# MinghanLi/MDQE_CVPR2023

Measured on AMD Instinct MI355X. Metric: frames/sec (eval-only) R50 OVIS 360p 4-frame clip, higher is better.
Workload: dtype f32; 1 GPU; R50_ovis_360 eval-only, H2D included: 120 synthetic 360x640 u8 frames/GPU/step from pinned host memory, 4-frame clips stride 1, 30-frame windows, one model(inputs) call per video; random-init weights, calibrated class logits (DESIGN.md §5); frames_per_gpu=120, instances_out=10, tracked_instances=7, gemm=exact fp32 MFMA, hw_queues=4, ranks_seen=1, parallelism=single GPU

## Files before the change

include/mdqe_hip.h:

```cpp
#ifndef MDQE_HIP_H
#define MDQE_HIP_H
#include <stdint.h>

#ifdef __cplusplus
extern "C" {
#endif

#define MDQE_OK 0
#define MDQE_EINVAL 1
#define MDQE_ELAUNCH 2
#define MDQE_ENULL 3
#define MDQE_ESTATE 4

#define MDQE_ACT_NONE 0
#define MDQE_ACT_RELU 1
#define MDQE_ACT_GELU 2
#define MDQE_ACT_SIGMOID 3
#define MDQE_ACT_TANH 4

#define MDQE_ABI_VERSION 6
int mdqe_abi_version(void);
int mdqe_version(void);
const char* mdqe_strerror(int code);

// ... 116 lines not shown
int mdqe_stem_conv_f32(const void* frames, int is_u8, long frame_stride, int NI, int h, int w, int Hp, int Wp,
                       const float* mean3_host, const float* std3_host, const float* wk, const float* bias, float* out,
                       void* stream);

int mdqe_maxpool3x3s2_nhwc_f32(const float* x, float* y, int NI, int H, int W, int C, void* stream);

int mdqe_upsample_nearest_add_nhwc_f32(const float* a, const float* b, float* y, int NI, int H, int W, int Hb, int Wb,
                                       int C, void* stream);

int mdqe_dwconv5x5_nhwc_f32(const float* x, const float* wt, const float* bias, float* y, int NI, int H, int W, int C,
                            int up2, const float* tw, const float* tb, void* stream);

int mdqe_dwconv5x5_c256_f32(const float* x, const float* wt, const float* bias, float* y, int NI, int H, int W, void* stream);
int mdqe_dwconv5x5_up2_c256_f32(const float* x, const float* wt, const float* bias, const float* tw, const float* tb, float* y,
                                int NI, int Hs, int Ws, void* stream);

int mdqe_trk_siou_f32(const float* saved, long saved_stride, int n_saved, const float* inp, long inp_stride,
                      int n_in, long n, float* out3, void* stream);
int mdqe_trk_accumulate_f32(float* sum, long sum_stride, float* cnt, long cnt_stride, const float* src,
                            long src_stride, long n, int nf, const int* r_host, const int* c_host, int count,
                            void* stream);
int mdqe_trk_siou_host_f32(const float* saved, long saved_stride, int n_saved, const float* inp, long inp_stride,
                           int n_in, long n, float* acc, unsigned* ticket, unsigned long long* out_host,
                           unsigned seq, void* stream);
int mdqe_trk_wait_counts(const unsigned long long* out_host, int n_out, unsigned seq, int spin_us, float* counts, void* stream);

int mdqe_trk_window_mean_f32(const float* sum, const float* cnt, long hw, int mem_len, int n, int nf, long f0,
                             float* out, void* stream);
int mdqe_trk_carry_f32(float* sum, float* cnt, long hw, int mem_len, int n, int k, long src0, float* carry, void* stream);

// ... 17 lines not shown
                            float* carry, float* out_cls, int* n, int* ln, void* stream);

int mdqe_clip_assoc_f32(const float* emb, int Q, int E, const int* fidx, int Bc, int T, int ct, float wdw, int nb,
                        int* idx_out, void* stream);
int mdqe_clip_gather_init_f32(const float* content, const float* coords, const int* fidx, const int* idx, int Bc, int T,
                              int Q, int C, int ct, float* x, float* ref, float* xinst, void* stream);
int mdqe_box_refine_f32(const float* delta, const float* prev, int Bc, int T, int Q, int t0, int t1, float* boxes,
                        float* ibox, void* stream);
int mdqe_add_rows_f32(const float* a, long lda, const float* b, long ldb, float* out, long ldo, long rows, int C, void* stream);
int mdqe_time_fuse_f32(const float* w, const float* x, int Bc, int T, int Q, int C, float* out, const float* pos,
                       float* out_plus_pos, void* stream);
int mdqe_box_head_refine_f32(const float* h, long ldh, const float* W, const float* bias, const float* prev, int Bc, int T, int Q, int K,
                             int t0, int t1, float* boxes, float* ibox, void* stream);
int mdqe_time_fuse_dot_f32(const float* xw, const float* wt, const float* bt, const float* src, int Bc, int T, int Q, int C, float* out,
                           void* stream);

int mdqe_clip_select_f32(const float* cls, const float* emb, int B, int Q, int K, int C, float thr, int max_keep,
                         int* order_ws, int* n_thr_ws, float* inv_norm_ws, float* sim_ws, int* kept, int* n_keep, void* stream);
long mdqe_dyn_mask_workspace_floats(int n_rows, int T, int H, int W);
int mdqe_dyn_mask_nms_f32(const float* coef, const int* kept, const float* feats, int B, int Q, int M, int T, int H, int W,
                          const int* row0_host, const int* n_host, const int* f0_host, float* logits, float* soft_h,
                          float* hard_h, float* part, float* gram, float* stats, float* mi, void* stream);
long mdqe_nms_workspace_floats(int n_max);
int mdqe_clip_finalize_f32(const float* cls, const float* emb, const int* kept, const float* stats, const float* mi, int B,
                           int Q, int K, int C, float thr, const int* row0_host, const int* n_host, int* sel, int* n_sel,
                           float* out, void* stream);
int mdqe_rows_gather_f32(const float* src, const int* idx_dev, int n, long len, float* out, void* stream);

int mdqe_mask_row_stats_f32(const float* logits, int n, int T, int H, int W, int t_step, float* stats5,
                            float* soft_h, float* hard_h, void* stream);
// ... 76 lines not shown
```

mdqe_cvpr2023_amd/_lib.py:

```python
import ctypes
import os
from ctypes import c_char_p, c_float, c_int, c_void_p

_HERE = os.path.dirname(os.path.abspath(__file__))
LIB_PATH = os.environ.get("MDQE_HIP_LIB") or os.path.join(_HERE, "csrc", "libmdqe_hip.so")

from ctypes import c_long
i, f, p, l = c_int, c_float, c_void_p, c_long

SIGNATURES = {
    "mdqe_msda_forward_f32": [p, p, p, p, p, i, i, i, i, i, i, i, p, p],
    "mdqe_msda_backward_f32": [p, p, p, p, p, p, i, i, i, i, i, i, i, p, p, p, p],
    "mdqe_msda_forward_f64": [p, p, p, p, p, i, i, i, i, i, i, i, p, p],
    "mdqe_msda_backward_f64": [p, p, p, p, p, p, i, i, i, i, i, i, i, p, p, p, p],
    "mdqe_msda_forward_grouped_f32": [p, p, p, p, p, i, i, i, i, i, i, i, i, f, p, p],
    "mdqe_msda_fused_f32": [p, l, l, p, p, l, p, l, p, l, i, i, p, p, p, p, i, i, i, i, i, i, i, f, p, l, l, p],
    "mdqe_trk_siou_f32": [p, l, i, p, l, i, l, p, p],
    "mdqe_trk_accumulate_f32": [p, l, p, l, p, l, l, i, p, p, i, p],
    "mdqe_trk_window_mean_f32": [p, p, l, i, i, i, l, p, p],
    "mdqe_trk_carry_f32": [p, p, l, i, i, i, l, p, p],
    "mdqe_lsap_f64": [p, i, i, i, p, p, p],
    "mdqe_tracker_create": [i, i, i, i, i, i, f, p],
    "mdqe_tracker_destroy": [p],
    "mdqe_tracker_state": [p, p, p, p],
    "mdqe_tracker_overlap": [p, i, i, p, p, p, p],
    "mdqe_tracker_decide": [p, i, i, i, p, p, p, p, p, p, p, p, p, p],
    "mdqe_tracker_result": [p, i, p, p, p, p],
    "mdqe_tracker_update": [p, p, p, l, i, i, i, p, p, p, p, l, p, p, p],
    "mdqe_tracker_update_many": [p, p, p, l, i, p, p, p, p, p, p, p, p, p, p, p, p],
    "mdqe_tracker_get_result": [p, i, p, p, l, p, p, p, p, p, p],
    "mdqe_clip_assoc_f32": [p, i, i, p, i, i, i, f, i, p, p],
    "mdqe_clip_gather_init_f32": [p, p, p, p, i, i, i, i, i, p, p, p, p],
    "mdqe_box_refine_f32": [p, p, i, i, i, i, i, p, p, p],
    "mdqe_add_rows_f32": [p, l, p, l, p, l, l, i, p],
    "mdqe_time_fuse_f32": [p, p, i, i, i, i, p, p, p, p],
    "mdqe_box_head_refine_f32": [p, l, p, p, p, i, i, i, i, i, i, p, p, p],
    "mdqe_time_fuse_dot_f32": [p, p, p, p, i, i, i, i, p, p],
    "mdqe_clip_select_f32": [p, p, i, i, i, i, f, i, p, p, p, p, p, p, p],
    "mdqe_dyn_mask_nms_f32": [p, p, p, i, i, i, i, i, i, p, p, p, p, p, p, p, p, p, p, p],
    "mdqe_clip_finalize_f32": [p, p, p, p, p, i, i, i, i, f, p, p, p, p, p, p],
    "mdqe_rows_gather_f32": [p, p, i, l, p, p],
    "mdqe_mha_small_f32": [p, l, p, l, p, l, i, i, i, i, p],
    "mdqe_query_select_f32": [p, i, i, i, i, i, p, p, p],
    "mdqe_sample_levels_mean_f32": [p, i, l, i, p, i, p, p, p, i, p, p],
    "mdqe_image_mask_stats_f32": [p, i, i, i, i, i, i, p, p],
    "mdqe_image_final_masks_u8": [p, i, p, i, i, i, i, i, i, i, p, p],
    "mdqe_final_masks_rle": [p, i, p, i, i, i, i, i, i, i, i, i, p, p, p],
    "mdqe_final_masks_u8": [p, i, p, i, i, i, i, i, i, i, i, p, l, i, p],
    "mdqe_final_masks_rle_geom": [p, i, p, i, i, i, i, i, i, i, i, i, p, p, p, p],
    "mdqe_final_masks_u8_geom": [p, i, p, i, i, i, i, i, i, i, i, p, l, i, p, p],
    "mdqe_final_label_map_u8": [p, i, p, i, i, i, i, i, i, i, i, p, i, p, p],
    "mdqe_render_overlay_u8": [p, i, l, i, i, p, i, i, i, p, i, i, p, i, p],
# ... 46 lines not shown
    "mdqe_gemm_ln_f32": [p, l, p, p, p, l, i, i, i, p, l, p, p, f, p],
    "mdqe_gemm_ln2_f32": [p, l, p, p, p, l, i, i, i, p, l, p, p, p, p, p, l, f, p],
    "mdqe_gemm_nt_side_f32": [p, l, p, p, p, l, i, i, i, p, p, i, p, p],
    "mdqe_gemm_nt_cat2_f32": [p, l, i, p, l, i, i, i, i, i, i, i, p, p, p, l, i, i, p],
    "mdqe_gemm_nt_pix_f32": [p, l, i, i, i, i, i, i, i, p, p, p, l, i, i, p],
    "mdqe_groupnorm_nhwc_f32": [p, l, l, p, l, l, i, i, i, i, p, p, f, i, p, p],
    "mdqe_resize_pil_bilinear_u8": [p, l, i, i, i, i, i, i, p, p, p, i, p, p, p, i, p, p],
    "mdqe_yuv420sp_to_rgb_u8": [p, l, l, p, l, l, i, i, i, i, i, i, i, p, p],
    "mdqe_stem_im2col_f32": [p, i, l, i, i, i, i, i, p, p, p, p],
    "mdqe_stem_conv_f32": [p, i, l, i, i, i, i, i, p, p, p, p, p, p],
    "mdqe_maxpool3x3s2_nhwc_f32": [p, p, i, i, i, i, p],
    "mdqe_upsample_nearest_add_nhwc_f32": [p, p, p, i, i, i, i, i, i, p],
    "mdqe_dwconv5x5_nhwc_f32": [p, p, p, p, i, i, i, i, i, p, p, p],
    "mdqe_dwconv5x5_c256_f32": [p, p, p, p, i, i, i, p],
    "mdqe_dwconv5x5_up2_c256_f32": [p, p, p, p, p, p, i, i, i, p],
}


ABI_VERSION = 6


class LibraryMissing(RuntimeError):
    pass


class MdqeError(RuntimeError):
    pass


_lib = None
# ... 71 lines not shown
```

mdqe_cvpr2023_amd/csrc/clip_ops.hip:

```cpp
#include "common.h"

#include <math.h>

template <int E>
__global__ void __launch_bounds__(64)
clip_assoc_kernel(const float* __restrict__ emb, const int* __restrict__ fidx, int T, int Q, int ct, float wdw, int nb,
                  int* __restrict__ idx) {
  extern __shared__ __attribute__((aligned(16))) float sE[];
  const int bt = blockIdx.y, b = bt / T, t = bt % T;
  const int k = blockIdx.x * 64 + threadIdx.x;
  const float* et = emb + (long)fidx[b * T + t] * Q * E;
  const float* ec = emb + (long)fidx[b * T + ct] * Q * E;
  for (int i = threadIdx.x; i < Q * (E / 4); i += 64)
    *reinterpret_cast<f32x4*>(sE + i * 4) = *reinterpret_cast<const f32x4*>(et + i * 4);
  __syncthreads();
  if (k >= Q) return;
  float c[E];
#pragma unroll
  for (int e = 0; e < E; e += 4) {
    const f32x4 v = *reinterpret_cast<const f32x4*>(ec + (long)k * E + e);
    c[e] = v[0]; c[e + 1] = v[1]; c[e + 2] = v[2]; c[e + 3] = v[3];
  }
  const float w = wdw * (float)abs(t - ct);
  const int ki = k / nb, kj = k % nb;
// ... 231 lines not shown
    }
  }
  if (lane == 0) *reinterpret_cast<f32x4*>(ibox + i * 4) = f32x4{(x0 + x1) / 2.f, (y0 + y1) / 2.f, x1 - x0, y1 - y0};
}

extern "C" int mdqe_box_head_refine_f32(const float* h, long ldh, const float* W, const float* bias, const float* prev, int Bc, int T,
                                        int Q, int K, int t0, int t1, float* boxes, float* ibox, void* stream) {
  MDQE_REQUIRE(Bc >= 0 && T > 0 && Q > 0 && K > 0 && K % 256 == 0 && ldh >= K && ldh % 4 == 0 && t0 >= 0 && t0 < t1);
  if (Bc == 0) return MDQE_OK;
  MDQE_CHECK_PTR(h); MDQE_CHECK_PTR(W); MDQE_CHECK_PTR(bias); MDQE_CHECK_PTR(prev); MDQE_CHECK_PTR(boxes); MDQE_CHECK_PTR(ibox);
  MDQE_REQUIRE((((uintptr_t)h | (uintptr_t)W | (uintptr_t)prev | (uintptr_t)boxes | (uintptr_t)ibox) & 15) == 0);
  mdqe_clear_error();
  const long n = (long)Bc * Q;
  hipLaunchKernelGGL(box_head_refine_kernel, dim3((unsigned)((n + 3) / 4)), dim3(256), 0, (hipStream_t)stream, h, ldh, W, bias, prev, T, Q, K,
                     t0, t1 < T ? t1 : T, n, boxes, ibox);
  return mdqe_launch_status();
}

__global__ void __launch_bounds__(256)
time_fuse_dot_kernel(const float* __restrict__ xw, const float* __restrict__ wt, const float* __restrict__ bt,
                     const float* __restrict__ src, int T, int Q, long n, float* __restrict__ out) {
  constexpr int C = 256, TMAX = 8;
  const int lane = threadIdx.x & 63;
  const long i = (long)blockIdx.x * 4 + (threadIdx.x >> 6);
  if (i >= n) return;
  const long b = i / Q;
  const int q = (int)(i % Q);
  const f32x4 w = *reinterpret_cast<const f32x4*>(wt + lane * 4);
  float tw[TMAX];
  float m = -INFINITY;
// ... 477 lines not shown
```

mdqe_cvpr2023_amd/engine.py:

```python
import contextlib
import math
import os
from types import SimpleNamespace as NS

import numpy as np
import torch
import torch.nn.functional as F

from . import ops
from .config import MDQEConfig
from .params import ALIASES, RESNET_BLOCKS, msda_dir_grid


def _fold_bn(sd, p, eps=1e-5):
    scale = sd[p + ".norm.weight"] * (sd[p + ".norm.running_var"] + eps).rsqrt()
    shift = sd[p + ".norm.bias"] - sd[p + ".norm.running_mean"] * scale
    return sd[p + ".weight"] * scale.view(-1, 1, 1, 1), shift


GEO_CACHE = max(1, int(os.environ.get("MDQE_GEO_CACHE", "16")))
STEM_FUSED = os.environ.get("MDQE_STEM_FUSED", "1") != "0"
SWIN_FUSED = os.environ.get("MDQE_SWIN_FUSED", "1") != "0"
RESNET_CAT = os.environ.get("MDQE_RESNET_CAT", "1") != "0"

# ... 296 lines not shown


def box_cxcywh_to_xyxy(b):
    cx, cy, w, h = b.unbind(-1)
    return torch.stack([cx - 0.5 * w, cy - 0.5 * h, cx + 0.5 * w, cy + 0.5 * h], -1)


def box_xyxy_to_cxcywh(b):
    x0, y0, x1, y1 = b.unbind(-1)
    return torch.stack([(x0 + x1) / 2, (y0 + y1) / 2, x1 - x0, y1 - y0], -1)


INST_STREAMS = {}
DEC_TWO_STREAMS = os.environ.get("MDQE_DEC_TWO_STREAMS", "1") != "0"
DEC_FUSED = os.environ.get("MDQE_DEC_FUSED", "1") != "0"


class Engine:
    def __init__(self, cfg: MDQEConfig, state_dict, device="cuda", backbone_fn=None, only_backbone=False):
        self.cfg = cfg
        self.P = Packed(state_dict, cfg, device, only_backbone=only_backbone)
        self.dev = self.P.dev
        self.backbone_fn = backbone_fn
        self._geo = {}
        self.precision_map = os.environ.get("MDQE_PRECISION_MAP", "")
        if self.precision_map not in ("", "reference", "autocast_f16"):
            raise ValueError("MDQE_PRECISION_MAP: '' (exact fp32 everywhere), 'reference' or 'autocast_f16', not %r" % self.precision_map)

    def amp(self):
        if self.precision_map == "reference" and self.dev.type == "cuda":
# ... 146 lines not shown
    def _mask_features(self, enc, geo, out=None):
        mh, cfg = self.P.mh, self.cfg
        NI, N, C = enc.shape
        lv = [enc[:, geo.starts[l]:geo.starts[l] + geo.hw[l]].view(NI, geo.shapes[l][0], geo.shapes[l][1], C) for l in range(3)]
        x = ops.conv2d_nhwc(lv[2], *mh.lay1, 1, 1)
        x = ops.groupnorm_nhwc(x, 8, *mh.gn1, act="gelu", out=x).view(x.shape)
        for i, f in ((2, lv[1]), (3, lv[0])):
            cur = ops.conv2d_nhwc(f, *getattr(mh, f"ad{i - 1}"), 1, 0)
            x = ops.upsample_nearest_add(cur, x, out=cur)
            x = ops.conv2d_nhwc(x, *getattr(mh, f"lay{i}"), 1, 1)
            x = ops.groupnorm_nhwc(x, 8, *getattr(mh, f"gn{i}"), act="gelu", out=x).view(x.shape)
        o1, o2 = mh.out_lay1, mh.out_lay2
        y = ops.dwconv5x5(x, o1.dw, o1.db)
        y = ops.linear(y.view(-1, C), o1.pw, o1.pb).view(x.shape)
        y = ops.groupnorm_nhwc(y, 32, o1.g, o1.beta, act="relu", out=y).view(x.shape)
        z = ops.dwconv5x5(y, o2.dw, o2.db, up2=True, tw=mh.tw, tb=mh.tb)
        Md = o2.pw.shape[0]
        if out is not None and (tuple(out.shape) != (NI, z.shape[1], z.shape[2], Md) or not out.is_contiguous()):
            raise RuntimeError("mask_features: out must be a contiguous [NI, Hm, Wm, M] tensor")
        z2 = ops.linear(z.view(-1, C), o2.pw, o2.pb, out=None if out is None else out.view(-1, Md)).view(NI, z.shape[1], z.shape[2], Md)
        return ops.groupnorm_nhwc(z2, 32 if Md % 32 == 0 else 24, o2.g, o2.beta, act="relu", out=z2).view(z2.shape)

    def _mlp(self, x, layers, last_act=None, out=None):
        n = len(layers)
        for i, (w, b) in enumerate(layers):
            x = ops.linear(x, w, b, act="gelu" if i < n - 1 else last_act, out=out if i == n - 1 else None)
        return x

    def frame_queries(self, enc, geo, out=None):
        cfg = self.cfg
        NI, N, C = enc.shape
        H, W = geo.shapes[0]
        nb = cfg.n_bins
        o_coords, o_content, o_emb = out if out is not None else (None, None, None)
        with self.amp():
# ... 34 lines not shown
    def decode_clips(self, cache, starts, T, geo, two_streams=True):
        P, cfg = self.P, self.cfg
        Bc = len(starts)
        fidx_h = np.asarray([[a + t for t in range(T)] for a in starts], dtype=np.int32).reshape(Bc, T)
        lo, hi = int(fidx_h.min()), int(fidx_h.max()) + 1
        if lo > 0 or hi < cache["content"].shape[0]:
            cache = {k: v[lo:hi] for k, v in cache.items() if k in ("coords", "content", "emb", "vals")}
            fidx_h = fidx_h - lo
        fidx = self._to_dev_i32(fidx_h)
        content, vals = cache["content"], cache["vals"]
        Q, C = content.shape[1], content.shape[2]
        nh, N = cfg.nheads, geo.N
        D, Tc = C // nh, cfg.n_frames
        ct = int((T - 1) / 2)
        idx = ops.clip_assoc(cache["emb"], fidx, ct, cfg.window_inter_frame_asso / 2, cfg.n_bins) if T > 1 else None
        x, ref, x_inst = ops.clip_gather_init(content, cache["coords"], fidx, idx, ct)
        BT = Bc * T
        fused = DEC_FUSED
        small = fused and C == 256

        def refine(z, prev, zn=None):
            z = ops.layernorm(z, *P.dec_norm) if zn is None else zn
            if small:
                h = ops.linear(ops.linear(z, *P.bbox_embed[0], act="gelu"), *P.bbox_embed[1], act="gelu")
                return ops.box_head_refine(h, *P.bbox_embed[2], prev, Bc, T, Q, t0, t1)
            return ops.box_refine(self._mlp(z, P.bbox_embed), prev, Bc, T, Q, t0, t1)

        def qkv(sa, z, box, B_):
            if fused:
                o = ops.linear_side(z, sa.wqkv, sa.bqkv_pos, box, sa.side_w, 2 * C)
                return ops.mha_small(o[:, :2 * C], o[:, 2 * C:], B_, Q, C, nh)
            zp = ops.add_rows(z, ops.linear(box, *P.p2p))
            return ops.mha_small(ops.linear(zp, sa.wqk, sa.bqk), ops.linear(z, sa.wv, sa.bv), B_, Q, C, nh)

        def qproj(m, z, box):
            if fused:
                return ops.linear_side(z, m.wq, m.bq_pos, box, m.side_w, m.wq.shape[0])
            return ops.linear(ops.add_rows(z, ops.linear(box, *P.p2p)), m.wq, m.bq)

        t0, t1 = max(ct - int((Tc - 1) / 2), 0), ct + Tc
        boxes, ibox = refine(x, ref)
        itv = max(int(T / Tc), 1)
        ts = max(ct - int((Tc - 1) / 2) * itv, 0)
        tca = list(range(ts, T, itv))[:Tc]
        tca = tca + [tca[-1]] * (Tc - len(tca))
        lv_sp = ([s[0] for s in geo.shapes], [s[1] for s in geo.shapes], geo.starts)
        lv_tp = ([s[0] for s in geo.shapes for _ in range(Tc)], [s[1] for s in geo.shapes for _ in range(Tc)],
                 [f * N + geo.starts[g] for g in range(len(geo.shapes)) for f in tca])
        LP = cfg.n_levels * cfg.dec_points
        TP = Tc * cfg.dec_points
        vals2 = vals.view(-1, vals.shape[-1])
        vidx_sp = fidx.view(-1)
        vidx_tp = self._to_dev_i32(fidx_h[:, 0])
        vi = 0
        main = torch.cuda.current_stream(self.dev) if self.dev.type == "cuda" else None
        two = DEC_TWO_STREAMS and two_streams and main is not None and len(P.dec) > 1
        if two:
            pool = INST_STREAMS
            side = pool.get(main.cuda_stream)
            if side is None:
                side = pool[main.cuda_stream] = torch.cuda.Stream(self.dev, priority=-1)
            side.wait_stream(main)
            hold = [x_inst]

        def inst_level(L, x, sx, x_inst, ibox, vi):
            if small:
                fq = ops.time_fuse_dot(x, *L.time_weights, sx, Bc, T, Q)
            else:
                fq = ops.time_fuse(ops.linear(x, *L.time_weights), sx, Bc, T, Q)
            if L.ta is not None:
                pr = qproj(L.ta, fq, ibox)
                a = ops.msda_fused(vals2[:, vi * C:(vi + 1) * C], pr[:, :2 * nh * TP], pr[:, 2 * nh * TP:], ibox.view(Bc, Q, 4), lv_tp,
                                   Bc, Q, nh, D, Tc, cfg.dec_points, mode=1, grid=P.grid_tp, groups=len(geo.shapes),
                                   scale=1.0 / len(geo.shapes), v_brows=N, vidx=vidx_tp)
                x_inst = ops.linear_ln(a, L.ta.wo, L.ta.bo, x_inst, *L.norm2_inst)
            else:
                x_inst = ops.layernorm(x_inst, *L.norm2_inst, res=fq)
            x_inst = ops.linear_ln(qkv(L.sai, x_inst, ibox, Bc), L.sai.wo, L.sai.bo, x_inst, *L.norm1_inst)
            hdn = ops.linear(x_inst, *L.linear1_inst, act="gelu")
            return ops.linear_ln(hdn, *L.linear2_inst, x_inst, *L.norm3_inst)

        for L in P.dec:
            pr = qproj(L.ca, x, boxes)
            a = ops.msda_fused(vals2[:, vi * C:(vi + 1) * C], pr[:, :2 * nh * LP], pr[:, 2 * nh * LP:], boxes.view(BT, Q, 4), lv_sp,
                               BT, Q, nh, D, cfg.n_levels, cfg.dec_points, mode=1, grid=P.grid_sp, v_brows=N, vidx=vidx_sp)
            vi += 1
            x = ops.linear_ln(a, L.ca.wo, L.ca.bo, x, *L.norm2)
            sx = x
            x = ops.linear_ln(qkv(L.sa, x, boxes, BT), L.sa.wo, L.sa.bo, x, *L.norm1)
            hdn = ops.linear(x, *L.linear1, act="gelu")
            xn = None
            if L is not P.dec[-1]:
                x, xn = ops.linear_ln(hdn, *L.linear2, x, *L.norm3, second=P.dec_norm)
            else:
                x = ops.linear_ln(hdn, *L.linear2, x, *L.norm3)
            vi_inst = vi
            if L.ta is not None:
                vi += 1
            if two:
                ev = torch.cuda.Event()
                ev.record(main)
                with torch.cuda.stream(side):
# ... 75 lines not shown
```

mdqe_cvpr2023_amd/ops.py:

```python
import contextlib
import os
import threading

import torch

from ._lib import check, cur_stream, lib, ptr, raw_stream

ACT = {"none": 0, None: 0, "relu": 1, "gelu": 2, "sigmoid": 3, "tanh": 4}

if os.environ.get("MDQE_MSDA_VARIANT"):
    check(lib.mdqe_debug_msda_variant(int(os.environ["MDQE_MSDA_VARIANT"])), "msda_variant")

if os.environ.get("MDQE_MSDA_DEC_STAGED"):
    check(lib.mdqe_debug_msda_dec_staged(int(os.environ["MDQE_MSDA_DEC_STAGED"])), "msda_dec_staged")

if os.environ.get("MDQE_GEMM_TILE_RULE"):
    check(lib.mdqe_debug_gemm_tile_rule(int(os.environ["MDQE_GEMM_TILE_RULE"])), "gemm_tile_rule")
if os.environ.get("MDQE_GEMM_STAGGER"):
    check(lib.mdqe_debug_gemm_stagger(int(os.environ["MDQE_GEMM_STAGGER"])), "gemm_stagger")

if os.environ.get("MDQE_MSDA_DEC_STAGE_KB"):
    check(lib.mdqe_debug_msda_dec_stage_kb(int(os.environ["MDQE_MSDA_DEC_STAGE_KB"])), "msda_dec_stage_kb")
if os.environ.get("MDQE_MSDA_TP_STAGED"):
    check(lib.mdqe_debug_msda_tp_staged(int(os.environ["MDQE_MSDA_TP_STAGED"])), "msda_tp_staged")
# ... 357 lines not shown
    out = torch.empty((NI, OH, OW, C), dtype=torch.float32, device=x.device)
    if C == 256 and DW_FAST:
        if up2:
            _chk(tw, "tw"); _chk(tb, "tb")
            check(lib.mdqe_dwconv5x5_up2_c256_f32(ptr(x), ptr(wt), ptr(bias), ptr(tw), ptr(tb), ptr(out), NI, H, W, cur_stream()),
                  "dwconv5x5_up2_c256")
        else:
            check(lib.mdqe_dwconv5x5_c256_f32(ptr(x), ptr(wt), ptr(bias), ptr(out), NI, H, W, cur_stream()), "dwconv5x5_c256")
        return out
    check(lib.mdqe_dwconv5x5_nhwc_f32(ptr(x), ptr(wt), ptr(bias), ptr(out), NI, OH, OW, C, int(up2), ptr(tw), ptr(tb),
                                      cur_stream()), "dwconv5x5")
    return out


DW_FAST = os.environ.get("MDQE_DW_FAST", "1") != "0"


def msda(value, shapes_dev, starts_dev, loc, attn, groups=1, scale=1.0, out=None):
    B, S, M, D = value.shape
    Q, L, P = loc.shape[1], loc.shape[3], loc.shape[4]
    if out is None:
        out = torch.empty((B, Q, M * D), dtype=torch.float32, device=value.device)
    check(lib.mdqe_msda_forward_grouped_f32(ptr(value), ptr(shapes_dev), ptr(starts_dev), ptr(loc), ptr(attn), B, S, M, D,
                                            groups, L, Q, P, scale, ptr(out), cur_stream()), "msda")
    return out


def msda_fused(value, offs, logits, ref, levels, B, Q, M, D, L, P, mode=0, grid=None, groups=1, scale=1.0,
               v_brows=None, out=None, vidx=None):
    import ctypes
# ... 539 lines not shown
    boxes = torch.empty(Bc * T * Q, 4, device=delta.device)
    ibox = torch.empty(Bc * Q, 4, device=delta.device)
    check(lib.mdqe_box_refine_f32(ptr(delta), ptr(prev), Bc, T, Q, t0, t1, ptr(boxes), ptr(ibox), cur_stream()), "box_refine")
    return boxes, ibox


def box_head_refine(h, w, b, prev, Bc, T, Q, t0, t1):
    _chk(h, "h"); _chk(w, "w"); _chk(b, "b"); _chk(prev, "prev")
    boxes = torch.empty(Bc * T * Q, 4, device=h.device)
    ibox = torch.empty(Bc * Q, 4, device=h.device)
    check(lib.mdqe_box_head_refine_f32(ptr(h), h.stride(0), ptr(w), ptr(b), ptr(prev), Bc, T, Q, h.shape[1], t0, t1, ptr(boxes), ptr(ibox),
                                       cur_stream()), "box_head_refine")
    return boxes, ibox


def time_fuse_dot(xw, wt, bt, src, Bc, T, Q):
    _chk(xw, "xw"); _chk(wt, "wt"); _chk(bt, "bt"); _chk(src, "src")
    C = src.shape[-1]
    out = torch.empty(Bc * Q, C, device=src.device)
    check(lib.mdqe_time_fuse_dot_f32(ptr(xw), ptr(wt), ptr(bt), ptr(src), Bc, T, Q, C, ptr(out), cur_stream()), "time_fuse_dot")
    return out


def add_rows(a, b, out=None):
    rows, C = a.shape
    if out is None:
        out = torch.empty(rows, C, device=a.device)
    check(lib.mdqe_add_rows_f32(ptr(a), a.stride(0), ptr(b), b.stride(0), ptr(out), out.stride(0), rows, C, cur_stream()), "add_rows")
    return out

# ... 74 lines not shown
```

Baseline: 855.2 frames/s.

## Fuse mask-head up2 dwconv with pointwise GEMM and dedupe first decoder layer

Adds a fused kernel that computes the 2x-upsampled depthwise 5x5 conv and immediately applies the pointwise projection via MFMA from LDS. This avoids writing and re-reading the full-resolution 256-channel intermediate. It also runs the first decoder layer's box refine and cross-attention once per unique frame, since overlapping clips repeat frames. A new gather kernel then expands those results into clip rows, removing redundant per-clip work at the cost of more code paths and a precondition that this is exact only because first-layer inputs are per-frame.

```diff
diff --git a/include/mdqe_hip.h b/include/mdqe_hip.h
--- a/include/mdqe_hip.h
+++ b/include/mdqe_hip.h
@@ -154,6 +154,8 @@
 int mdqe_dwconv5x5_c256_f32(const float* x, const float* wt, const float* bias, float* y, int NI, int H, int W, void* stream);
 int mdqe_dwconv5x5_up2_c256_f32(const float* x, const float* wt, const float* bias, const float* tw, const float* tb, float* y,
                                 int NI, int Hs, int Ws, void* stream);
+int mdqe_dwup2_pw_f32(const float* x, const float* wt, const float* bias, const float* tw, const float* tb, const float* pw,
+                      const float* pb, float* out, long ldo, int NI, int Hs, int Ws, int Md, void* stream);
 
 int mdqe_trk_siou_f32(const float* saved, long saved_stride, int n_saved, const float* inp, long inp_stride,
                       int n_in, long n, float* out3, void* stream);
@@ -201,6 +203,8 @@
                              int t0, int t1, float* boxes, float* ibox, void* stream);
 int mdqe_time_fuse_dot_f32(const float* xw, const float* wt, const float* bt, const float* src, int Bc, int T, int Q, int C, float* out,
                            void* stream);
+int mdqe_clip_gather_prefix_f32(const float* x1, const float* box0, const float* content, const int* fidx, const int* idx, int Bc, int T,
+                                int Q, int C, int ct, int t0, int t1, float* x, float* boxes, float* xinst, float* ibox, void* stream);
 
 int mdqe_clip_select_f32(const float* cls, const float* emb, int B, int Q, int K, int C, float thr, int max_keep,
                          int* order_ws, int* n_thr_ws, float* inv_norm_ws, float* sim_ws, int* kept, int* n_keep, void* stream);
diff --git a/mdqe_cvpr2023_amd/_lib.py b/mdqe_cvpr2023_amd/_lib.py
--- a/mdqe_cvpr2023_amd/_lib.py
+++ b/mdqe_cvpr2023_amd/_lib.py
@@ -36,6 +36,7 @@
     "mdqe_time_fuse_f32": [p, p, i, i, i, i, p, p, p, p],
     "mdqe_box_head_refine_f32": [p, l, p, p, p, i, i, i, i, i, i, p, p, p],
     "mdqe_time_fuse_dot_f32": [p, p, p, p, i, i, i, i, p, p],
+    "mdqe_clip_gather_prefix_f32": [p, p, p, p, p, i, i, i, i, i, i, i, p, p, p, p, p],
     "mdqe_clip_select_f32": [p, p, i, i, i, i, f, i, p, p, p, p, p, p, p],
     "mdqe_dyn_mask_nms_f32": [p, p, p, i, i, i, i, i, i, p, p, p, p, p, p, p, p, p, p, p],
     "mdqe_clip_finalize_f32": [p, p, p, p, p, i, i, i, i, f, p, p, p, p, p, p],
@@ -112,6 +113,7 @@
     "mdqe_dwconv5x5_nhwc_f32": [p, p, p, p, i, i, i, i, i, p, p, p],
     "mdqe_dwconv5x5_c256_f32": [p, p, p, p, i, i, i, p],
     "mdqe_dwconv5x5_up2_c256_f32": [p, p, p, p, p, p, i, i, i, p],
+    "mdqe_dwup2_pw_f32": [p, p, p, p, p, p, p, p, l, i, i, i, i, p],
 }
 
 
diff --git a/mdqe_cvpr2023_amd/csrc/clip_ops.hip b/mdqe_cvpr2023_amd/csrc/clip_ops.hip
--- a/mdqe_cvpr2023_amd/csrc/clip_ops.hip
+++ b/mdqe_cvpr2023_amd/csrc/clip_ops.hip
@@ -269,6 +269,53 @@
   const long n = (long)Bc * Q;
   hipLaunchKernelGGL(box_head_refine_kernel, dim3((unsigned)((n + 3) / 4)), dim3(256), 0, (hipStream_t)stream, h, ldh, W, bias, prev, T, Q, K,
                      t0, t1 < T ? t1 : T, n, boxes, ibox);
+  return mdqe_launch_status();
+}
+
+__global__ void __launch_bounds__(256)
+clip_gather_prefix_kernel(const float* __restrict__ x1, const float* __restrict__ box0, const float* __restrict__ content,
+                          const int* __restrict__ fidx, const int* __restrict__ idx, int T, int Q, int C, int ct, int t0, int t1, long rows,
+                          float* __restrict__ x, float* __restrict__ boxes, float* __restrict__ xinst, float* __restrict__ ibox) {
+  const long r = (long)blockIdx.x * 4 + (threadIdx.x >> 6);
+  if (r >= rows) return;
+  const int lane = threadIdx.x & 63;
+  const int k = (int)(r % Q);
+  const long bt = r / Q;
+  const int t = (int)(bt % T);
+  const long b = bt / T;
+  const int q = idx ? idx[r] : k;
+  const long src = (long)fidx[bt] * Q + q;
+  const float* s = x1 + src * C;
+  float* d = x + r * C;
+  for (int c = lane * 4; c < C; c += 256) *reinterpret_cast<f32x4*>(d + c) = *reinterpret_cast<const f32x4*>(s + c);
+  if (lane == 0) *reinterpret_cast<f32x4*>(boxes + r * 4) = *reinterpret_cast<const f32x4*>(box0 + src * 4);
+  if (t != ct) return;
+  const float* si = content + ((long)fidx[bt] * Q + k) * C;
+  float* di = xinst + (b * Q + k) * C;
+  for (int c = lane * 4; c < C; c += 256) *reinterpret_cast<f32x4*>(di + c) = *reinterpret_cast<const f32x4*>(si + c);
+  float x0 = INFINITY, y0 = INFINITY, xb = -INFINITY, yb = -INFINITY;
+  for (int tt = t0; tt < t1; ++tt) {
+    const long rr = (b * T + tt) * Q + k;
+    const f32x4 o = *reinterpret_cast<const f32x4*>(box0 + ((long)fidx[b * T + tt] * Q + (idx ? idx[rr] : k)) * 4);
+    const float ax = fminf(fmaxf(o[0] - 0.5f * o[2], 0.f), 1.f), ay = fminf(fmaxf(o[1] - 0.5f * o[3], 0.f), 1.f);
+    const float bx = fminf(fmaxf(o[0] + 0.5f * o[2], 0.f), 1.f), by = fminf(fmaxf(o[1] + 0.5f * o[3], 0.f), 1.f);
+    x0 = fminf(x0, ax); y0 = fminf(y0, ay); xb = fmaxf(xb, bx); yb = fmaxf(yb, by);
+  }
+  if (lane == 0) *reinterpret_cast<f32x4*>(ibox + (b * Q + k) * 4) = f32x4{(x0 + xb) / 2.f, (y0 + yb) / 2.f, xb - x0, yb - y0};
+}
+
+extern "C" int mdqe_clip_gather_prefix_f32(const float* x1, const float* box0, const float* content, const int* fidx, const int* idx,
+                                           int Bc, int T, int Q, int C, int ct, int t0, int t1, float* x, float* boxes, float* xinst,
+                                           float* ibox, void* stream) {
+  MDQE_REQUIRE(Bc >= 0 && T > 0 && Q > 0 && C > 0 && C % 4 == 0 && ct >= 0 && ct < T && t0 >= 0 && t0 < t1);
+  if (Bc == 0) return MDQE_OK;
+  MDQE_CHECK_PTR(x1); MDQE_CHECK_PTR(box0); MDQE_CHECK_PTR(content); MDQE_CHECK_PTR(fidx); MDQE_CHECK_PTR(x); MDQE_CHECK_PTR(boxes);
+  MDQE_CHECK_PTR(xinst); MDQE_CHECK_PTR(ibox);
+  MDQE_REQUIRE((((uintptr_t)x1 | (uintptr_t)box0 | (uintptr_t)content | (uintptr_t)x | (uintptr_t)boxes | (uintptr_t)xinst | (uintptr_t)ibox) & 15) == 0);
+  mdqe_clear_error();
+  const long rows = (long)Bc * T * Q;
+  hipLaunchKernelGGL(clip_gather_prefix_kernel, dim3((unsigned)((rows + 3) / 4)), dim3(256), 0, (hipStream_t)stream, x1, box0, content, fidx,
+                     idx, T, Q, C, ct, t0, t1 < T ? t1 : T, rows, x, boxes, xinst, ibox);
   return mdqe_launch_status();
 }
 
diff --git a/mdqe_cvpr2023_amd/csrc/maskhead_out.hip b/mdqe_cvpr2023_amd/csrc/maskhead_out.hip
--- /dev/null
+++ b/mdqe_cvpr2023_amd/csrc/maskhead_out.hip
@@ -0,0 +1,302 @@
+#include "common.h"
+#include "gemm_device.h"
+#include <type_traits>
+
+namespace {
+__device__ __forceinline__ f32x4 ld4(const float* p) { return *reinterpret_cast<const f32x4*>(p); }
+constexpr int C = 256;
+constexpr int TILE_PITCH = 260;
+constexpr int TILE_FLOATS = 32 * TILE_PITCH;
+
+template <int NC>
+__device__ __forceinline__ void quad_taps(const f32x4 (&X)[3][NC], const int c0, const bool (&rok)[3], const f32x4 (&w)[25], f32x4& o00,
+                                          f32x4& o01, f32x4& o10, f32x4& o11) {
+  o00 = f32x4{0.f, 0.f, 0.f, 0.f}; o01 = o00; o10 = o00; o11 = o00;
+#pragma unroll
+  for (int r = 0; r < 3; ++r) {
+    if (!rok[r]) continue;
+#pragma unroll
+    for (int c = 0; c < 3; ++c) o00 += X[r][c0 + c] * w[(2 * r) * 5 + 2 * c];
+#pragma unroll
+    for (int c = 1; c < 3; ++c) o01 += X[r][c0 + c] * w[(2 * r) * 5 + 2 * c - 1];
+    if (r >= 1) {
+#pragma unroll
+      for (int c = 0; c < 3; ++c) o10 += X[r][c0 + c] * w[(2 * r - 1) * 5 + 2 * c];
+#pragma unroll
+      for (int c = 1; c < 3; ++c) o11 += X[r][c0 + c] * w[(2 * r - 1) * 5 + 2 * c - 1];
+    }
+  }
+}
+
+__device__ __forceinline__ f32x4 border_const(int hh, int ww, int H, int W, const f32x4 (&w)[25], f32x4 bv, f32x4 tbv) {
+  f32x4 s = {0.f, 0.f, 0.f, 0.f};
+#pragma unroll
+  for (int kh = 0; kh < 5; ++kh) {
+    const int ih = hh - 2 + kh;
+    if (ih < 0 || ih >= H) continue;
+#pragma unroll
+    for (int kw = 0; kw < 5; ++kw) {
+      const int iw = ww - 2 + kw;
+      if (iw >= 0 && iw < W) s += w[kh * 5 + kw];
+    }
+  }
+  return bv + tbv * s;
+}
+}
+
+__global__ void __launch_bounds__(256)
+dwup2_pw_kernel(const float* __restrict__ x, const float* __restrict__ wt, const float* __restrict__ bias, const float* __restrict__ tw,
+                const float* __restrict__ tb, const float* __restrict__ pw, const float* __restrict__ pb, float* __restrict__ out, long ldo,
+                int NI, int Hs, int Ws, int Md) {
+  extern __shared__ __attribute__((aligned(16))) float lds[];
+  const int lane = threadIdx.x & 63;
+  const int wave = __builtin_amdgcn_readfirstlane(threadIdx.x >> 6);
+  const long wid = (long)blockIdx.x * 4 + wave, nw = (long)gridDim.x * 4;
+  const int lr = lane & 31, lh = lane >> 5;
+  const int H = 2 * Hs, W = 2 * Ws;
+  float* const sW = lds + 4 * TILE_FLOATS;
+  for (int i = threadIdx.x; i < 25 * C / 4; i += 256) *reinterpret_cast<f32x4*>(sW + i * 4) = ld4(wt + i * 4);
+  __syncthreads();
+  const float* const wl = sW + lane * 4;
+  auto tap = [&](int t) __attribute__((always_inline)) { return ld4(wl + t * C); };
+  const f32x4 twv = ld4(tw + lane * 4);
+  f32x4 cin;
+  {
+    f32x4 wall = {0.f, 0.f, 0.f, 0.f};
+#pragma unroll
+    for (int t = 0; t < 25; ++t) wall += tap(t);
+    cin = ld4(bias + lane * 4) + ld4(tb + lane * 4) * wall;
+  }
+
+  f32x4 bf[16][2];
+#pragma unroll
+  for (int kt = 0; kt < 16; ++kt)
+#pragma unroll
+    for (int h = 0; h < 2; ++h)
+      bf[kt][h] = lr < Md ? ld4(pw + (long)lr * C + kt * 16 + h * 8 + lh * 4) : f32x4{0.f, 0.f, 0.f, 0.f};
+  float* const sA = lds + wave * TILE_FLOATS;
+  const int c4 = lane & 7, r8 = lane >> 3;
+  const f32x4 pbv = c4 * 4 < Md ? ld4(pb + c4 * 4) : f32x4{0.f, 0.f, 0.f, 0.f};
+
+  const int nseg = (Ws + 7) >> 3;
+  const long ntiles = (long)NI * Hs * nseg;
+  f32x4 X[3][10];
+  auto load_tile = [&](long tile) __attribute__((always_inline)) {
+    const int b0 = (int)(tile % nseg) * 8;
+    const long ra = tile / nseg;
+    const int a = (int)(ra % Hs);
+    const long r0 = ra - a;
+#pragma unroll
+    for (int r = 0; r < 3; ++r) {
+      const int ia = min(max(a - 1 + r, 0), Hs - 1);
+      const float* row = x + ((r0 + ia) * Ws) * C + lane * 4;
+#pragma unroll
+      for (int c = 0; c < 10; ++c) X[r][c] = ld4(row + (long)min(max(b0 - 1 + c, 0), Ws - 1) * C);
+    }
+  };
+  if (wid < ntiles) load_tile(wid);
+  for (long tile = wid; tile < ntiles; tile += nw) {
+    const int b0 = (int)(tile % nseg) * 8;
+    const long ra = tile / nseg;
+    const int a = (int)(ra % Hs);
+    const long img = ra / Hs;
+    const bool rok[3] = {a >= 1, true, a + 1 < Hs};
+    const bool edge = a == 0 || a == Hs - 1 || b0 == 0 || b0 + 8 >= Ws;
+    if (edge) {
+#pragma unroll
+      for (int c = 0; c < 10; ++c)
+        if (b0 - 1 + c < 0 || b0 - 1 + c >= Ws) {
+#pragma unroll
+          for (int r = 0; r < 3; ++r) X[r][c] = f32x4{0.f, 0.f, 0.f, 0.f};
+        }
+      for (int qi = 0; qi < 8; ++qi) {
+        float* d = sA + (qi * 4) * TILE_PITCH + lane * 4;
+#pragma unroll
+        for (int j = 0; j < 4; ++j) *reinterpret_cast<f32x4*>(d + j * TILE_PITCH) = cin;
+      }
+      const bool rb = a == 0 || a == Hs - 1;
+#pragma unroll 1
+      for (int kind = 0; kind < 3; ++kind) {
+        int bq;
+        if (kind == 0) { if (b0 != 0) continue; bq = 0; }
+        else if (kind == 1) { bq = Ws - 1; if (bq == 0 || bq < b0 || bq >= b0 + 8) continue; }
+        else { if (!rb || Ws < 3) continue; bq = 1; }
+        f32x4 w[25];
+#pragma unroll
+        for (int t = 0; t < 25; ++t) w[t] = tap(t);
+        const f32x4 bv = ld4(bias + lane * 4), tbv = ld4(tb + lane * 4);
+        const f32x4 k00 = border_const(2 * a, 2 * bq, H, W, w, bv, tbv), k01 = border_const(2 * a, 2 * bq + 1, H, W, w, bv, tbv);
+        const f32x4 k10 = border_const(2 * a + 1, 2 * bq, H, W, w, bv, tbv), k11 = border_const(2 * a + 1, 2 * bq + 1, H, W, w, bv, tbv);
+#pragma unroll 1
+        for (int qi = 0; qi < 8; ++qi) {
+          const int b = b0 + qi;
+          if (b >= Ws) break;
+          if (kind == 0 ? b != 0 : kind == 1 ? b != Ws - 1 : (b == 0 || b == Ws - 1)) continue;
+          float* d = sA + (qi * 4) * TILE_PITCH + lane * 4;
+          *reinterpret_cast<f32x4*>(d) = k00; *reinterpret_cast<f32x4*>(d + TILE_PITCH) = k01;
+          *reinterpret_cast<f32x4*>(d + 2 * TILE_PITCH) = k10; *reinterpret_cast<f32x4*>(d + 3 * TILE_PITCH) = k11;
+        }
+      }
+    }
+#pragma unroll
+    for (int h4 = 0; h4 < 2; ++h4) {
+      f32x4 o00[4], o01[4], o10[4], o11[4];
+#pragma unroll
+      for (int q = 0; q < 4; ++q) { o00[q] = f32x4{0.f, 0.f, 0.f, 0.f}; o01[q] = o00[q]; o10[q] = o00[q]; o11[q] = o00[q]; }
+#pragma unroll
+      for (int r = 0; r < 3; ++r) {
+        if (!rok[r]) continue;
+#pragma unroll
+        for (int c = 0; c < 3; ++c) {
+          const f32x4 wa = tap((2 * r) * 5 + 2 * c);
+#pragma unroll
+          for (int q = 0; q < 4; ++q) o00[q] += X[r][h4 * 4 + q + c] * wa;
+          if (c >= 1) {
+            const f32x4 wb = tap((2 * r) * 5 + 2 * c - 1);
+#pragma unroll
+            for (int q = 0; q < 4; ++q) o01[q] += X[r][h4 * 4 + q + c] * wb;
+          }
+          if (r >= 1) {
+            const f32x4 wc = tap((2 * r - 1) * 5 + 2 * c);
+#pragma unroll
+            for (int q = 0; q < 4; ++q) o10[q] += X[r][h4 * 4 + q + c] * wc;
+            if (c >= 1) {
+              const f32x4 wd = tap((2 * r - 1) * 5 + 2 * c - 1);
+#pragma unroll
+              for (int q = 0; q < 4; ++q) o11[q] += X[r][h4 * 4 + q + c] * wd;
+            }
+          }
+        }
+      }
+#pragma unroll
+      for (int q = 0; q < 4; ++q) {
+        float* d = sA + ((h4 * 4 + q) * 4) * TILE_PITCH + lane * 4;
+        f32x4 c00 = cin, c01 = cin, c10 = cin, c11 = cin;
+        if (edge) { c00 = ld4(d); c01 = ld4(d + TILE_PITCH); c10 = ld4(d + 2 * TILE_PITCH); c11 = ld4(d + 3 * TILE_PITCH); }
+        *reinterpret_cast<f32x4*>(d) = c00 + twv * o00[q];
+        *reinterpret_cast<f32x4*>(d + TILE_PITCH) = c01 + twv * o01[q];
+        *reinterpret_cast<f32x4*>(d + 2 * TILE_PITCH) = c10 + twv * o10[q];
+        *reinterpret_cast<f32x4*>(d + 3 * TILE_PITCH) = c11 + twv * o11[q];
+      }
+    }
+    if (tile + nw < ntiles) load_tile(tile + nw);
+    asm volatile("s_waitcnt lgkmcnt(0)" ::: "memory");
+    __builtin_amdgcn_wave_barrier();
+    f32x16 acc;
+#pragma unroll
+    for (int r = 0; r < 16; ++r) acc[r] = 0.f;
+    const float* fa = sA + lr * TILE_PITCH + lh * 4;
+    f32x4 af[4];
+#pragma unroll
+    for (int i = 0; i < 4; ++i) af[i] = ld4(fa + (i >> 1) * 16 + (i & 1) * 8);
+    __builtin_amdgcn_sched_barrier(0);
+#pragma unroll
+    for (int i = 0; i < 32; ++i) {
+#pragma unroll
+      for (int s = 0; s < 4; ++s) acc = __builtin_amdgcn_mfma_f32_32x32x2f32(af[i & 3][s], bf[i >> 1][i & 1][s], acc, 0, 0, 0);
+      __builtin_amdgcn_sched_barrier(0);
+      if (i + 4 < 32) af[i & 3] = ld4(fa + ((i + 4) >> 1) * 16 + ((i + 4) & 1) * 8);
+      __builtin_amdgcn_sched_barrier(0);
+    }
+    asm volatile("s_waitcnt lgkmcnt(0)" ::: "memory");
+    __builtin_amdgcn_wave_barrier();
+#pragma unroll
+    for (int r = 0; r < 16; ++r) sA[gemm_acc_row(r, lh) * 32 + lr] = acc[r];
+    asm volatile("s_waitcnt lgkmcnt(0)" ::: "memory");
+    __builtin_amdgcn_wave_barrier();
+#pragma unroll
+    for (int it = 0; it < 4; ++it) {
+      const int prow = it * 8 + r8;
+      f32x4 v = ld4(sA + prow * 32 + c4 * 4);
+      v += pbv;
+      const int b = b0 + (prow >> 2);
+      if (b < Ws && c4 * 4 < Md) {
+        const long pix = (img * H + 2 * a + ((prow >> 1) & 1)) * W + 2 * b + (prow & 1);
+        *reinterpret_cast<f32x4*>(out + pix * ldo + c4 * 4) = v;
+      }
+    }
+    asm volatile("s_waitcnt lgkmcnt(0)" ::: "memory");
+    __builtin_amdgcn_wave_barrier();
+  }
+}
+
+__global__ void __launch_bounds__(256)
+dwup2_dot_kernel(const float* __restrict__ x, const float* __restrict__ wt, const float* __restrict__ bias, const float* __restrict__ tw,
+                 const float* __restrict__ tb, const float* __restrict__ pw, const float* __restrict__ pb, float* __restrict__ out, long ldo,
+                 int NI, int Hs, int Ws, int Md) {
+  const int lane = threadIdx.x & 63;
+  const long wid = (long)blockIdx.x * 4 + (threadIdx.x >> 6), nw = (long)gridDim.x * 4;
+  const int H = 2 * Hs, W = 2 * Ws;
+  f32x4 w[25];
+#pragma unroll
+  for (int t = 0; t < 25; ++t) w[t] = ld4(wt + t * C + lane * 4);
+  const f32x4 bv = ld4(bias + lane * 4), twv = ld4(tw + lane * 4), tbv = ld4(tb + lane * 4);
+  f32x4 wall = {0.f, 0.f, 0.f, 0.f};
+#pragma unroll
+  for (int t = 0; t < 25; ++t) wall += w[t];
+  const f32x4 cin = bv + tbv * wall;
+  const long total = (long)NI * Hs * Ws;
+  for (long i = wid; i < total; i += nw) {
+    const int b = (int)(i % Ws); const long ra = i / Ws;
+    const int a = (int)(ra % Hs); const long img = ra / Hs;
+    const bool rok[3] = {a >= 1, true, a + 1 < Hs};
+    f32x4 X[3][3];
+#pragma unroll
+    for (int r = 0; r < 3; ++r) {
+      const float* row = x + ((ra - 1 + r) * Ws) * C + lane * 4;
+#pragma unroll
+      for (int c = 0; c < 3; ++c) {
+        const int ib = b - 1 + c;
+        X[r][c] = (rok[r] && ib >= 0 && ib < Ws) ? ld4(row + (long)ib * C) : f32x4{0.f, 0.f, 0.f, 0.f};
+      }
+    }
+    f32x4 o00, o01, o10, o11;
+    quad_taps(X, 0, rok, w, o00, o01, o10, o11);
+    f32x4 c00 = cin, c01 = cin, c10 = cin, c11 = cin;
+    if (a == 0 || a == Hs - 1 || b == 0 || b == Ws - 1) {
+      c00 = border_const(2 * a, 2 * b, H, W, w, bv, tbv); c01 = border_const(2 * a, 2 * b + 1, H, W, w, bv, tbv);
+      c10 = border_const(2 * a + 1, 2 * b, H, W, w, bv, tbv); c11 = border_const(2 * a + 1, 2 * b + 1, H, W, w, bv, tbv);
+    }
+    const f32x4 zz[4] = {c00 + twv * o00, c01 + twv * o01, c10 + twv * o10, c11 + twv * o11};
+    float res[4] = {0.f, 0.f, 0.f, 0.f};
+    for (int n = 0; n < Md; ++n) {
+      const f32x4 wn = ld4(pw + (long)n * C + lane * 4);
+      const float bn = pb[n];
+#pragma unroll
+      for (int j = 0; j < 4; ++j) {
+        float v = fmaf(zz[j][3], wn[3], fmaf(zz[j][2], wn[2], fmaf(zz[j][1], wn[1], fmaf(zz[j][0], wn[0], 0.f))));
+#pragma unroll
+        for (int sft = 1; sft < 64; sft <<= 1) v += __shfl_xor(v, sft, 64);
+        if (lane == n) res[j] = v + bn;
+      }
+    }
+    if (lane < Md) {
+      float* o = out + ((img * H + 2 * a) * W + 2 * b) * ldo;
+      o[lane] = res[0]; o[ldo + lane] = res[1]; o[(long)W * ldo + lane] = res[2]; o[(long)W * ldo + ldo + lane] = res[3];
+    }
+  }
+}
+
+extern "C" int mdqe_dwup2_pw_f32(const float* x, const float* wt, const float* bias, const float* tw, const float* tb, const float* pw,
+                                 const float* pb, float* out, long ldo, int NI, int Hs, int Ws, int Md, void* stream) {
+  MDQE_REQUIRE(NI >= 0 && Hs > 0 && Ws > 0 && Md > 0 && Md <= 32 && Md % 4 == 0 && ldo >= Md && ldo % 4 == 0);
+  if (NI == 0) return MDQE_OK;
+  MDQE_CHECK_PTR(x); MDQE_CHECK_PTR(wt); MDQE_CHECK_PTR(bias); MDQE_CHECK_PTR(tw); MDQE_CHECK_PTR(tb); MDQE_CHECK_PTR(pw); MDQE_CHECK_PTR(pb);
+  MDQE_CHECK_PTR(out);
+  MDQE_REQUIRE((((uintptr_t)x | (uintptr_t)wt | (uintptr_t)bias | (uintptr_t)tw | (uintptr_t)tb | (uintptr_t)pw | (uintptr_t)pb |
+                 (uintptr_t)out) & 15) == 0);
+  mdqe_clear_error();
+  hipStream_t st = (hipStream_t)stream;
+  if (Md <= 8) {
+    const long total = (long)NI * Hs * Ws;
+    long nd = (total + 3) / 4; if (nd > 256 * 8) nd = 256 * 8;
+    hipLaunchKernelGGL(dwup2_dot_kernel, dim3((unsigned)nd), dim3(256), 0, st, x, wt, bias, tw, tb, pw, pb, out, ldo, NI, Hs, Ws, Md);
+    return mdqe_launch_status();
+  }
+  const long ntiles = (long)NI * Hs * ((Ws + 7) / 8);
+  long nb = (ntiles + 3) / 4; if (nb > 256) nb = 256;
+  const int smem = (4 * TILE_FLOATS + 25 * C) * (int)sizeof(float);
+  if (mdqe_allow_lds(reinterpret_cast<const void*>(dwup2_pw_kernel), smem) != hipSuccess) return MDQE_ELAUNCH;
+  hipLaunchKernelGGL(dwup2_pw_kernel, dim3((unsigned)nb), dim3(256), smem, st, x, wt, bias, tw, tb, pw, pb, out, ldo, NI, Hs, Ws, Md);
+  return mdqe_launch_status();
+}
diff --git a/mdqe_cvpr2023_amd/engine.py b/mdqe_cvpr2023_amd/engine.py
--- a/mdqe_cvpr2023_amd/engine.py
+++ b/mdqe_cvpr2023_amd/engine.py
@@ -334,6 +334,7 @@
 INST_STREAMS = {}
 DEC_TWO_STREAMS = os.environ.get("MDQE_DEC_TWO_STREAMS", "1") != "0"
 DEC_FUSED = os.environ.get("MDQE_DEC_FUSED", "1") != "0"
+DEC_PREFIX = os.environ.get("MDQE_DEC_PREFIX", "1") != "0"
 
 
 class Engine:
@@ -510,11 +511,15 @@
         y = ops.dwconv5x5(x, o1.dw, o1.db)
         y = ops.linear(y.view(-1, C), o1.pw, o1.pb).view(x.shape)
         y = ops.groupnorm_nhwc(y, 32, o1.g, o1.beta, act="relu", out=y).view(x.shape)
-        z = ops.dwconv5x5(y, o2.dw, o2.db, up2=True, tw=mh.tw, tb=mh.tb)
         Md = o2.pw.shape[0]
-        if out is not None and (tuple(out.shape) != (NI, z.shape[1], z.shape[2], Md) or not out.is_contiguous()):
+        Hm, Wm = 2 * y.shape[1], 2 * y.shape[2]
+        if out is not None and (tuple(out.shape) != (NI, Hm, Wm, Md) or not out.is_contiguous()):
             raise RuntimeError("mask_features: out must be a contiguous [NI, Hm, Wm, M] tensor")
-        z2 = ops.linear(z.view(-1, C), o2.pw, o2.pb, out=None if out is None else out.view(-1, Md)).view(NI, z.shape[1], z.shape[2], Md)
+        if ops.dwup2_pw_ok(y, o2.pw):
+            z2 = ops.dwup2_pw(y, o2.dw, o2.db, mh.tw, mh.tb, o2.pw, o2.pb, out=out)
+        else:
+            z = ops.dwconv5x5(y, o2.dw, o2.db, up2=True, tw=mh.tw, tb=mh.tb)
+            z2 = ops.linear(z.view(-1, C), o2.pw, o2.pb, out=None if out is None else out.view(-1, Md)).view(NI, Hm, Wm, Md)
         return ops.groupnorm_nhwc(z2, 32 if Md % 32 == 0 else 24, o2.g, o2.beta, act="relu", out=z2).view(z2.shape)
 
     def _mlp(self, x, layers, last_act=None, out=None):
@@ -579,17 +584,17 @@
         D, Tc = C // nh, cfg.n_frames
         ct = int((T - 1) / 2)
         idx = ops.clip_assoc(cache["emb"], fidx, ct, cfg.window_inter_frame_asso / 2, cfg.n_bins) if T > 1 else None
-        x, ref, x_inst = ops.clip_gather_init(content, cache["coords"], fidx, idx, ct)
         BT = Bc * T
         fused = DEC_FUSED
         small = fused and C == 256
 
-        def refine(z, prev, zn=None):
+        def refine(z, prev, zn=None, rows=None):
+            B_, T_, a, b = (Bc, T, t0, t1) if rows is None else rows
             z = ops.layernorm(z, *P.dec_norm) if zn is None else zn
             if small:
                 h = ops.linear(ops.linear(z, *P.bbox_embed[0], act="gelu"), *P.bbox_embed[1], act="gelu")
-                return ops.box_head_refine(h, *P.bbox_embed[2], prev, Bc, T, Q, t0, t1)
-            return ops.box_refine(self._mlp(z, P.bbox_embed), prev, Bc, T, Q, t0, t1)
+                return ops.box_head_refine(h, *P.bbox_embed[2], prev, B_, T_, Q, a, b)
+            return ops.box_refine(self._mlp(z, P.bbox_embed), prev, B_, T_, Q, a, b)
 
         def qkv(sa, z, box, B_):
             if fused:
@@ -604,7 +609,6 @@
             return ops.linear(ops.add_rows(z, ops.linear(box, *P.p2p)), m.wq, m.bq)
 
         t0, t1 = max(ct - int((Tc - 1) / 2), 0), ct + Tc
-        boxes, ibox = refine(x, ref)
         itv = max(int(T / Tc), 1)
         ts = max(ct - int((Tc - 1) / 2) * itv, 0)
         tca = list(range(ts, T, itv))[:Tc]
@@ -618,6 +622,21 @@
         vidx_sp = fidx.view(-1)
         vidx_tp = self._to_dev_i32(fidx_h[:, 0])
         vi = 0
+        Fu = content.shape[0]
+        prefix = DEC_PREFIX and Fu < BT and ops.get_gemm_precision() == "f32"
+        if prefix:
+            L0 = P.dec[0]
+            c2 = content.view(Fu * Q, C)
+            ref0 = torch.nn.functional.pad(cache["coords"].reshape(Fu * Q, 2), (0, 2), value=0.1)
+            box0, _ = refine(c2, ref0, rows=(Fu, 1, 0, 1))
+            pr = qproj(L0.ca, c2, box0)
+            a = ops.msda_fused(vals2[:, :C], pr[:, :2 * nh * LP], pr[:, 2 * nh * LP:], box0.view(Fu, Q, 4), lv_sp,
+                               Fu, Q, nh, D, cfg.n_levels, cfg.dec_points, mode=1, grid=P.grid_sp, v_brows=N)
+            x1 = ops.linear_ln(a, L0.ca.wo, L0.ca.bo, c2, *L0.norm2)
+            x, boxes, x_inst, ibox = ops.clip_gather_prefix(x1, box0, content, fidx, idx, ct, t0, t1)
+        else:
+            x, ref, x_inst = ops.clip_gather_init(content, cache["coords"], fidx, idx, ct)
+            boxes, ibox = refine(x, ref)
         main = torch.cuda.current_stream(self.dev) if self.dev.type == "cuda" else None
         two = DEC_TWO_STREAMS and two_streams and main is not None and len(P.dec) > 1
         if two:
@@ -646,11 +665,12 @@
             return ops.linear_ln(hdn, *L.linear2_inst, x_inst, *L.norm3_inst)
 
         for L in P.dec:
-            pr = qproj(L.ca, x, boxes)
-            a = ops.msda_fused(vals2[:, vi * C:(vi + 1) * C], pr[:, :2 * nh * LP], pr[:, 2 * nh * LP:], boxes.view(BT, Q, 4), lv_sp,
-                               BT, Q, nh, D, cfg.n_levels, cfg.dec_points, mode=1, grid=P.grid_sp, v_brows=N, vidx=vidx_sp)
+            if not (prefix and L is P.dec[0]):
+                pr = qproj(L.ca, x, boxes)
+                a = ops.msda_fused(vals2[:, vi * C:(vi + 1) * C], pr[:, :2 * nh * LP], pr[:, 2 * nh * LP:], boxes.view(BT, Q, 4), lv_sp,
+                                   BT, Q, nh, D, cfg.n_levels, cfg.dec_points, mode=1, grid=P.grid_sp, v_brows=N, vidx=vidx_sp)
+                x = ops.linear_ln(a, L.ca.wo, L.ca.bo, x, *L.norm2)
             vi += 1
-            x = ops.linear_ln(a, L.ca.wo, L.ca.bo, x, *L.norm2)
             sx = x
             x = ops.linear_ln(qkv(L.sa, x, boxes, BT), L.sa.wo, L.sa.bo, x, *L.norm1)
             hdn = ops.linear(x, *L.linear1, act="gelu")
diff --git a/mdqe_cvpr2023_amd/ops.py b/mdqe_cvpr2023_amd/ops.py
--- a/mdqe_cvpr2023_amd/ops.py
+++ b/mdqe_cvpr2023_amd/ops.py
@@ -395,6 +395,30 @@
 
 
 DW_FAST = os.environ.get("MDQE_DW_FAST", "1") != "0"
+MASKHEAD_FUSED = os.environ.get("MDQE_MASKHEAD_FUSED", "1") != "0"
+
+
+def dwup2_pw_ok(x, pw):
+    return (MASKHEAD_FUSED and DW_FAST and x.shape[-1] == 256 and pw.shape[0] % 4 == 0 and pw.shape[0] <= 32
+            and get_gemm_precision() == "f32")
+
+
+def dwup2_pw(x, wt, bias, tw, tb, pw, pb, out=None):
+    for t, n in ((x, "x"), (wt, "wt"), (bias, "bias"), (tw, "tw"), (tb, "tb"), (pw, "pw"), (pb, "pb")):
+        _chk(t, n)
+    NI, H, W, C = x.shape
+    Md = pw.shape[0]
+    if C != 256 or pw.shape[1] != 256 or Md % 4 or Md > 32:
+        raise RuntimeError("dwup2_pw: C == 256, Md % 4 == 0, Md <= 32 required")
+    if out is None:
+        out = torch.empty((NI, 2 * H, 2 * W, Md), dtype=torch.float32, device=x.device)
+    ldo = out.stride(2)
+    if (tuple(out.shape) != (NI, 2 * H, 2 * W, Md) or out.dtype != torch.float32 or not out.is_cuda or out.stride(3) != 1
+            or out.stride(1) != 2 * W * ldo or (NI > 1 and out.stride(0) != 4 * H * W * ldo)):
+        raise RuntimeError("dwup2_pw: out must be a CUDA fp32 [NI,2H,2W,Md] view with one pixel pitch")
+    check(lib.mdqe_dwup2_pw_f32(ptr(x), ptr(wt), ptr(bias), ptr(tw), ptr(tb), ptr(pw), ptr(pb), ptr(out), ldo, NI, H, W, Md, cur_stream()),
+          "dwup2_pw")
+    return out
 
 
 def msda(value, shapes_dev, starts_dev, loc, attn, groups=1, scale=1.0, out=None):
@@ -964,6 +988,21 @@
     return boxes, ibox
 
 
+def clip_gather_prefix(x1, box0, content, fidx, idx, ct, t0, t1):
+    _chk(x1, "x1"); _chk(box0, "box0"); _chk(content, "content"); _chk(fidx, "fidx", torch.int32); _chk(idx, "idx", torch.int32)
+    Bc, T = fidx.shape
+    F, Q, C = content.shape
+    if x1.shape != (F * Q, C) or box0.shape != (F * Q, 4) or (idx is not None and idx.numel() != Bc * T * Q):
+        raise RuntimeError("clip_gather_prefix: x1 [F*Q, C], box0 [F*Q, 4], idx [Bc, T, Q] for content [F, Q, C] required")
+    x = torch.empty(Bc * T * Q, C, device=content.device)
+    boxes = torch.empty(Bc * T * Q, 4, device=content.device)
+    xi = torch.empty(Bc * Q, C, device=content.device)
+    ibox = torch.empty(Bc * Q, 4, device=content.device)
+    check(lib.mdqe_clip_gather_prefix_f32(ptr(x1), ptr(box0), ptr(content), ptr(fidx), ptr(idx), Bc, T, Q, C, ct, t0, t1, ptr(x), ptr(boxes),
+                                          ptr(xi), ptr(ibox), cur_stream()), "clip_gather_prefix")
+    return x, boxes, xi, ibox
+
+
 def time_fuse_dot(xw, wt, bt, src, Bc, T, Q):
     _chk(xw, "xw"); _chk(wt, "wt"); _chk(bt, "bt"); _chk(src, "src")
     C = src.shape[-1]
```

Result: no change. 857.7 frames/s (median of 2 runs) (+0.3%).
